# Xinjie-Q/Boosting-NeRV

Hardware: AMD Instinct MI355X
Metric: train frames/sec (higher is better)
Workload: dtype fp32; 1 GPU; NeRV-boost 1.5M (1489577 params, fc_dim 30) train step on a synthetic Bunny-shaped clip 132x3x720x1280: decoder fwd + Fusion10_freq + bwd + fused Adan; frames resident in HBM; global_batch=1, per_gpu_batch=1, parallelism=dp1, hipgraph=True, rccl_ranks=0, collective_in_graph=False

## Files before the change

boosting_nerv_amd/csrc/loss.hip:

```cpp
#include "common.h"
#include "launch.h"
#include <vector>
#include <math.h>
#include <string.h>
#include <map>
#include <mutex>

namespace {

constexpr int NSB = 512;

__device__ __forceinline__ void diff_stats_body(const float* __restrict__ p, const float* __restrict__ t, float* __restrict__ part, int n_per_sample, const int bx, const int b) {
    const float* pp = p + (size_t)b * n_per_sample;
    const float* tt = t + (size_t)b * n_per_sample;
    float s1 = 0.f, s2 = 0.f;
    constexpr int STR = NSB * 256;
    int i = bx * 256 + threadIdx.x;
    for (; i + 3 * STR < n_per_sample; i += 4 * STR) {
        float d[4];
#pragma unroll
        for (int u = 0; u < 4; ++u) d[u] = pp[i + u * STR] - tt[i + u * STR];
#pragma unroll
        for (int u = 0; u < 4; ++u) { s1 += fabsf(d[u]); s2 = fmaf(d[u], d[u], s2); }
    }
// ... 77 lines not shown
        const int oy = (int)(r % Ho);
        const size_t pl = r / Ho;
        const int iy = 2 * oy - ph, ix = 2 * ox - pw;
        const float* xp = x + pl * H * W;
        float s = 0.f;
#pragma unroll
        for (int dy = 0; dy < 2; ++dy)
#pragma unroll
            for (int dx = 0; dx < 2; ++dx) {
                const int yy = iy + dy, xx = ix + dx;
                if (yy >= 0 && yy < H && xx >= 0 && xx < W) s += xp[(size_t)yy * W + xx];
            }
        y[i] = 0.25f * s;
    }
}

struct PyrArgs { const float* src[2]; float* dst[2][LV]; int H[LV], W[LV]; int planes; int vec2; };
__device__ __forceinline__ void pyramid_body(const PyrArgs& a, const int bx, const int by, const int bz) {
    __shared__ float s1[16][17], s2[8][9], s3[4][5];
    const int img = bz & 1, pl = bz >> 1;
    const float* x = a.src[img] + (size_t)pl * a.H[0] * a.W[0];
    const int tid = threadIdx.x, ty = tid >> 4, tx = tid & 15;
    {
        const int oy = by * 16 + ty, ox = bx * 16 + tx;
        float v = 0.f;
        if (oy < a.H[1] && ox < a.W[1]) {
            const float* p0 = x + (size_t)(2 * oy) * a.W[0] + 2 * ox;
            const float* p1 = p0 + a.W[0];
            float2 r0, r1;
            if (a.vec2) {
                r0 = *reinterpret_cast<const float2*>(p0);
                r1 = *reinterpret_cast<const float2*>(p1);
            } else {
                r0 = float2{p0[0], p0[1]};
                r1 = float2{p1[0], p1[1]};
            }
            v = 0.25f * (((r0.x + r0.y) + r1.x) + r1.y);
            a.dst[img][1][((size_t)pl * a.H[1] + oy) * a.W[1] + ox] = v;
        }
        s1[ty][tx] = v;
    }
    __syncthreads();
    if (tid < 64) {
        const int y = tid >> 3, xx = tid & 7, oy = by * 8 + y, ox = bx * 8 + xx;
        const float v = 0.25f * (((s1[2 * y][2 * xx] + s1[2 * y][2 * xx + 1]) + s1[2 * y + 1][2 * xx]) + s1[2 * y + 1][2 * xx + 1]);
        if (oy < a.H[2] && ox < a.W[2]) a.dst[img][2][((size_t)pl * a.H[2] + oy) * a.W[2] + ox] = v;
        s2[y][xx] = v;
    }
    __syncthreads();
    if (tid < 16) {
        const int y = tid >> 2, xx = tid & 3, oy = by * 4 + y, ox = bx * 4 + xx;
        const float v = 0.25f * (((s2[2 * y][2 * xx] + s2[2 * y][2 * xx + 1]) + s2[2 * y + 1][2 * xx]) + s2[2 * y + 1][2 * xx + 1]);
        if (oy < a.H[3] && ox < a.W[3]) a.dst[img][3][((size_t)pl * a.H[3] + oy) * a.W[3] + ox] = v;
        s3[y][xx] = v;
    }
    __syncthreads();
    if (tid < 4) {
        const int y = tid >> 1, xx = tid & 1, oy = by * 2 + y, ox = bx * 2 + xx;
        const float v = 0.25f * (((s3[2 * y][2 * xx] + s3[2 * y][2 * xx + 1]) + s3[2 * y + 1][2 * xx]) + s3[2 * y + 1][2 * xx + 1]);
        if (oy < a.H[4] && ox < a.W[4]) a.dst[img][4][((size_t)pl * a.H[4] + oy) * a.W[4] + ox] = v;
    }
}
__global__ __launch_bounds__(256) void pyramid_kernel(const PyrArgs a) { pyramid_body(a, blockIdx.x, blockIdx.y, blockIdx.z); }

struct SsimArgs {
    const float* X; const float* Y;
    float* partial;
    const float* coef;
    float coef_k;
    const float* dcoarse;
    float* dX;
    float* G;
    int H, W, Hc, Wc, ph, pw;
    int tiles_x, tiles_y;
    float C1, C2;
    float k_l1, k_l2;
    int acc;
    Win win;
};

typedef float pk2 __attribute__((ext_vector_type(2)));
__device__ __forceinline__ pk2 pk_fma(pk2 a, pk2 b, pk2 c) { return __builtin_elementwise_fma(a, b, c); }

__device__ __forceinline__ void ssim_fwd_body(const SsimArgs& a, const bool LAST, const int bx, const int by, const int bc, const int nbc) {
#pragma clang fp contract(off)
    constexpr int WH = STH + HW_, WW = STW + HW_;
    __shared__ pk2 sXY[WH][WW];
    __shared__ pk2 sV01[STH][WW], sV23[STH][WW];
    __shared__ float sV4[STH][WW];
    __shared__ float red[4];
    const int tid = threadIdx.x;
    const int oy0 = by * STH, ox0 = bx * STW;
    const float* X = a.X + (size_t)bc * a.H * a.W;
    const float* Y = a.Y + (size_t)bc * a.H * a.W;
    {
        constexpr int NLD = (WH * WW + 255) / 256;
        pk2 ld[NLD];
#pragma unroll
        for (int u = 0; u < NLD; ++u) {
            const int i = tid + u * 256;
            const int r = i / WW, c = i - r * WW;
            const int y = oy0 + r, x = ox0 + c;
            const bool in = i < WH * WW && y < a.H && x < a.W;
            ld[u] = pk2{in ? X[(size_t)y * a.W + x] : 0.f, in ? Y[(size_t)y * a.W + x] : 0.f};
        }
#pragma unroll
        for (int u = 0; u < NLD; ++u) {
            const int i = tid + u * 256;
            if (i < WH * WW) (&sXY[0][0])[i] = ld[u];
        }
    }
    __syncthreads();
    for (int i = tid; i < STH * WW; i += 256) {
        const int r = i / WW, c = i - r * WW;
        pk2 v01 = {0.f, 0.f}, v23 = {0.f, 0.f};
        float v4 = 0.f;
#pragma unroll
        for (int k = 0; k < WS_; ++k) {
            const float g = a.win.g[k];
            const pk2 gg = {g, g}, xy = sXY[r + k][c];
            v01 = pk_fma(gg, xy, v01); v23 = pk_fma(gg, xy * xy, v23); v4 = fmaf(g, xy.x * xy.y, v4);
        }
        sV01[r][c] = v01; sV23[r][c] = v23; sV4[r][c] = v4;
    }
    __syncthreads();
    float acc = 0.f;
    const int Hv = a.H - HW_, Wv = a.W - HW_;
    for (int i = tid; i < STH * STW; i += 256) {
        const int r = i / STW, c = i - r * STW;
        pk2 m = {0.f, 0.f}, e = {0.f, 0.f};
        float exy = 0.f;
#pragma unroll
        for (int k = 0; k < WS_; ++k) {
            const float g = a.win.g[k];
            const pk2 gg = {g, g};
            m = pk_fma(gg, sV01[r][c + k], m); e = pk_fma(gg, sV23[r][c + k], e); exy = fmaf(g, sV4[r][c + k], exy);
        }
        const float m1 = m.x, m2 = m.y, exx = e.x, eyy = e.y;
        if (oy0 + r < Hv && ox0 + c < Wv) {
            const float m11 = m1 * m1, m22 = m2 * m2, m12 = m1 * m2;
            const float s1 = exx - m11, s2 = eyy - m22, s12 = exy - m12;
            const float B2 = s1 + s2 + a.C2;
            const float cs = (2.f * s12 + a.C2) / B2;
            float lum = 1.f;
            if (LAST) { lum = (2.f * m12 + a.C1) / (m11 + m22 + a.C1); acc += lum * cs; }
            else acc += cs;
            if (a.G) {
                const float dxy0 = 2.f * __builtin_amdgcn_rcpf(B2);
                float dm = dxy0 * (m1 * cs - m2), dxx = -0.5f * cs * dxy0, dxy = dxy0;
                if (LAST) {
                    const float B1 = m11 + m22 + a.C1;
                    dm = (2.f * __builtin_amdgcn_rcpf(B1)) * (m2 - m1 * lum) * cs + lum * dm;
                    dxx *= lum; dxy *= lum;
                }
                const size_t plane = (size_t)a.H * a.W, o = (size_t)bc * plane + (size_t)(oy0 + r) * a.W + (ox0 + c);
                const size_t mstride = (size_t)nbc * plane;
                a.G[o] = dm; a.G[mstride + o] = dxx; a.G[2 * mstride + o] = dxy;
            }
        }
    }
    acc = wave_sum(acc);
    if ((tid & 63) == 0) red[tid >> 6] = acc;
    __syncthreads();
    if (tid == 0) a.partial[(size_t)bc * (a.tiles_x * a.tiles_y) + by * a.tiles_x + bx] = red[0] + red[1] + red[2] + red[3];
}
struct Tile3 { int x, y, z; };
__device__ __forceinline__ Tile3 xcd_tile3() {
    const int gx = (int)gridDim.x, gy = (int)gridDim.y;
    const int lb = xcd_remap((int)(blockIdx.x + gridDim.x * (blockIdx.y + gridDim.y * blockIdx.z)), (int)(gridDim.x * gridDim.y * gridDim.z));
    const int z = lb / (gx * gy), r = lb - z * (gx * gy);
    return Tile3{r % gx, r / gx, z};
}
template <bool LAST>
__global__ __launch_bounds__(256) void ssim_fwd_kernel(const SsimArgs a) { const Tile3 t = xcd_tile3(); ssim_fwd_body(a, LAST, t.x, t.y, t.z, gridDim.z); }

struct SsimAllArgs { SsimArgs lv[LV]; int first[LV + 1]; };
__global__ __launch_bounds__(256) void ssim_fwd_all_kernel(const SsimAllArgs a) {
    const int lb = xcd_remap((int)(blockIdx.x + gridDim.x * blockIdx.y), (int)(gridDim.x * gridDim.y));
    const int gbx = lb % (int)gridDim.x, gby = lb / (int)gridDim.x;
    int l = 0;
#pragma unroll
    for (int k = 1; k < LV; ++k) if (gbx >= a.first[k]) l = k;
    const int t = gbx - a.first[l];
    const int bx = t % a.lv[l].tiles_x, by = t / a.lv[l].tiles_x;
    ssim_fwd_body(a.lv[l], l == LV - 1, bx, by, gby, gridDim.y);
}

struct CoefArgs {
    const float* partial[LV];
    int tiles[LV];
    float inv_nvalid[LV];
    float weights[LV];
    float* msval;
    float* coef;
    int BC;
    float chain;
};
__device__ __forceinline__ double tile_sum_d(const float* __restrict__ part, const int nt) {
    const int lane = threadIdx.x & 63;
    double s = 0.0;
    for (int i0 = lane; i0 < nt; i0 += 8 * 64) {
        float v[8];
#pragma unroll
        for (int u = 0; u < 8; ++u) { const int i = i0 + u * 64; v[u] = i < nt ? part[i] : 0.f; }
#pragma unroll
        for (int u = 0; u < 8; ++u) if (i0 + u * 64 < nt) s += (double)v[u];
    }
    return wave_sum_d(s);
}
__device__ __forceinline__ void ms_coef_body(const CoefArgs& a, const int bc) {
    const int lane = threadIdx.x & 63, nw = (int)blockDim.x >> 6;
    __shared__ float stat[LV];
    for (int l = threadIdx.x >> 6; l < LV; l += nw) {
        const double s = tile_sum_d(a.partial[l] + (size_t)bc * a.tiles[l], a.tiles[l]);
        if (lane == 0) stat[l] = (float)(s * (double)a.inv_nvalid[l]);
    }
    __syncthreads();
    if (threadIdx.x == 0) {
        float P = 1.f;
        for (int k = 0; k < LV; ++k) P *= powf(fmaxf(stat[k], 0.f), a.weights[k]);
        a.msval[bc] = P;
        for (int k = 0; k < LV; ++k)
            a.coef[(size_t)k * a.BC + bc] = stat[k] > 0.f ? a.chain * a.weights[k] * (P / stat[k]) * a.inv_nvalid[k] : 0.f;
    }
}
__global__ __launch_bounds__(320) void ms_coef_kernel(const CoefArgs a) { ms_coef_body(a, blockIdx.x); }

struct CoarseChain { const float* own[LV]; int H[LV], W[LV], ph[LV], pw[LV]; int n; };
constexpr int SSIM_BWD_LDS = 3 * (2 * STH + HW_) * (STW + HW_);
template <bool LEVEL0>
__device__ __forceinline__ void ssim_bwd_body(const SsimArgs& a, const CoarseChain* cc, float* lds, const int bx, const int by, const int bc, const int nbc) {
    constexpr int GH = STH + HW_, GW = STW + HW_;
    pk2 (*sG01)[GW] = reinterpret_cast<pk2 (*)[GW]>(lds);
    pk2 (*sA01)[GW] = reinterpret_cast<pk2 (*)[GW]>(lds + 2 * GH * GW);
    float (*sG2)[GW] = reinterpret_cast<float (*)[GW]>(lds + 2 * GH * GW + 2 * STH * GW);
    float (*sA2)[GW] = reinterpret_cast<float (*)[GW]>(lds + 3 * GH * GW + 2 * STH * GW);
    const int tid = threadIdx.x;
    const int py0 = by * STH, px0 = bx * STW;
    const int wy0 = py0 - HW_, wx0 = px0 - HW_;
    const int Hv = a.H - HW_, Wv = a.W - HW_;
    const size_t plane = (size_t)a.H * a.W, mstride = (size_t)nbc * plane;
    const float* Gp = a.G + (size_t)bc * plane;
    {
        constexpr int NLD = (GH * GW + 255) / 256;
        float l0[NLD], l1[NLD], l2[NLD];
#pragma unroll
        for (int u = 0; u < NLD; ++u) {
            const int i = tid + u * 256;
            const int r = i / GW, c = i - r * GW;
            const int oy = wy0 + r, ox = wx0 + c;
            l0[u] = 0.f; l1[u] = 0.f; l2[u] = 0.f;
            if (i < GH * GW && oy >= 0 && oy < Hv && ox >= 0 && ox < Wv) {
                const size_t o = (size_t)oy * a.W + ox;
                l0[u] = Gp[o]; l1[u] = Gp[mstride + o]; l2[u] = Gp[2 * mstride + o];
            }
        }
#pragma unroll
        for (int u = 0; u < NLD; ++u) {
            const int i = tid + u * 256;
            if (i < GH * GW) { (&sG01[0][0])[i] = pk2{l0[u], l1[u]}; (&sG2[0][0])[i] = l2[u]; }
        }
    }
    __syncthreads();
    for (int i = tid; i < STH * GW; i += 256) {
        const int r = i / GW, c = i - r * GW;
        pk2 a01 = {0.f, 0.f};
        float a2 = 0.f;
#pragma unroll
// ... 40 lines not shown
        }
        if (LEVEL0) {
            const float df = xv - yv;
            const float sg = (df > 0.f) ? 1.f : ((df < 0.f) ? -1.f : 0.f);
            d += a.k_l1 * sg + a.k_l2 * df;
        }
        float* dst = a.dX + ((size_t)bc * a.H + y) * a.W + x;
        *dst = (LEVEL0 && a.acc) ? d + *dst : d;
    }
}
template <bool LEVEL0>
__global__ __launch_bounds__(256) void ssim_bwd_from_g_kernel(const SsimArgs a) {
    __shared__ __attribute__((aligned(16))) float sl[SSIM_BWD_LDS];
    const Tile3 t = xcd_tile3(); ssim_bwd_body<LEVEL0>(a, nullptr, sl, t.x, t.y, t.z, gridDim.z);
}
__global__ __launch_bounds__(256) void ssim_bwd_level0_chain_kernel(const SsimArgs a, const CoarseChain cc) {
    __shared__ __attribute__((aligned(16))) float sl[SSIM_BWD_LDS];
    const Tile3 t = xcd_tile3(); ssim_bwd_body<true>(a, &cc, sl, t.x, t.y, t.z, gridDim.z);
}
__device__ __forceinline__ void ssim_bwd_coarse_body(const SsimAllArgs& a, float* lds, const int lin, const int gx, const int nbc) {
    const int lb = xcd_remap(lin, gx * nbc);
    const int gbx = lb % gx, gby = lb / gx;
    int l = 1;
#pragma unroll
    for (int k = 2; k < LV; ++k) if (gbx >= a.first[k]) l = k;
    const int t = gbx - a.first[l];
    const int tx = cdiv_d(a.lv[l].W, STW);
    ssim_bwd_body<false>(a.lv[l], nullptr, lds, t % tx, t / tx, gby, nbc);
}
__global__ __launch_bounds__(256) void ssim_bwd_coarse_all_kernel(const SsimAllArgs a) {
    __shared__ __attribute__((aligned(16))) float sl[SSIM_BWD_LDS];
    ssim_bwd_coarse_body(a, sl, (int)(blockIdx.x + gridDim.x * blockIdx.y), (int)gridDim.x, (int)gridDim.y);
}

#include "fft_body.h"
__global__ __launch_bounds__(256) void fft_rows_fwd_kernel(const FftArgs a) { fft_rows_fwd_body(a, blockIdx.x); }
__global__ __launch_bounds__(256) void fft_cols_kernel(const FftArgs a) {
    const int lb = xcd_remap((int)(blockIdx.x + gridDim.x * blockIdx.y), (int)(gridDim.x * gridDim.y));
    fft_cols_body(a, lb % (int)gridDim.x, lb / (int)gridDim.x, gridDim.x);
}
__global__ __launch_bounds__(256) void fft_rows_adj_kernel(const FftArgs a) { fft_rows_adj_body(a, blockIdx.x); }

struct FinalArgs {
    const float* stats_part;
    const float* msval;
    const float* fft_part;
    float* loss_out; float* stats_out;
    int B, C, n_per_sample, ncolblk;
    float c_l1, c_l2, c_ms, c_fft;
};
__device__ __forceinline__ void loss_final_body(const FinalArgs& a) {
    const int lane = threadIdx.x;
    double total = 0.0;
    for (int b = 0; b < a.B; ++b) {
        double s1 = 0.0, s2 = 0.0;
        for (int k = lane; k < NSB; k += 64) { s1 += (double)a.stats_part[((size_t)b * NSB + k) * 2]; s2 += (double)a.stats_part[((size_t)b * NSB + k) * 2 + 1]; }
        s1 = wave_sum_d(s1); s2 = wave_sum_d(s2);
        double l = (double)a.c_l1 * (s1 / a.n_per_sample) + (double)a.c_l2 * (s2 / a.n_per_sample);
        double ms = 0.0;
        if (a.msval) {
            for (int c = 0; c < a.C; ++c) ms += (double)a.msval[b * a.C + c];
            ms /= a.C;
            l += (double)a.c_ms * (1.0 - ms);
        }
        if (a.fft_part) {
            double f = 0.0;
            const int nf = a.C * a.ncolblk;
            for (int k = lane; k < nf; k += 64) f += (double)a.fft_part[(size_t)b * nf + k];
            f = wave_sum_d(f);
            l += (double)a.c_fft * f / (2.0 * (double)a.n_per_sample);
        }
        if (lane == 0) {
            float* so = a.stats_out + b * BNERV_LOSS_STATS;
            so[0] = (float)l; so[1] = (float)s1; so[2] = (float)s2; so[3] = (float)ms;
            const float mse = (float)(s2 / (double)a.n_per_sample);
            so[4] = -10.0f * log10f(mse + 1e-9f);
        }
        total += l;
    }
    if (lane == 0) a.loss_out[0] = (float)(total / a.B);
}
__global__ __launch_bounds__(64) void loss_final_kernel(const FinalArgs a) { loss_final_body(a); }

struct LossHeadArgs { FftArgs f; PyrArgs p; const float* pred; const float* target; float* stats_part; int nps, n_fft, n_pyr, pyr_gx, pyr_gy; };
__global__ __launch_bounds__(256) void loss_head_kernel(const LossHeadArgs a) {
    int b = blockIdx.x;
    if (b < a.n_fft) { fft_rows_fwd_body(a.f, b); return; }
    b -= a.n_fft;
    if (b < a.n_pyr) { const int bx = b % a.pyr_gx, r = b / a.pyr_gx; pyramid_body(a.p, bx, r % a.pyr_gy, r / a.pyr_gy); return; }
    b -= a.n_pyr;
    diff_stats_body(a.pred, a.target, a.stats_part, a.nps, b % NSB, b / NSB);
}
struct LossMidArgs { FftArgs f; CoefArgs c; int ncolblk, n_cols; };
__global__ __launch_bounds__(256) void loss_mid_kernel(const LossMidArgs a) {
    const int b = blockIdx.x;
    if (b < a.n_cols) {
        const int xcd = b & 7, k = b >> 3, per = a.n_cols >> 3, extra = a.n_cols & 7;
        const int lb = xcd * per + min(xcd, extra) + k;
        fft_cols_body(a.f, lb % a.ncolblk, lb / a.ncolblk, a.ncolblk);
    } else ms_coef_body(a.c, b - a.n_cols);
}
struct LossTailArgs { SsimArgs s; CoarseChain cc; FinalArgs fin; int gx, gy, n0, BC; };
__global__ __launch_bounds__(256) void loss_tail_kernel(const LossTailArgs a) {
    __shared__ __attribute__((aligned(16))) float sl[SSIM_BWD_LDS];
    if ((int)blockIdx.x < a.n0) { const int b = xcd_remap((int)blockIdx.x, a.n0); const int bx = b % a.gx, r = b / a.gx; ssim_bwd_body<true>(a.s, &a.cc, sl, bx, r % a.gy, r / a.gy, a.BC); }
    else if (threadIdx.x < 64) loss_final_body(a.fin);
}
struct LossCoarseArgs { FftArgs f; SsimAllArgs s; int n_adj, gx, BC; };
__global__ __launch_bounds__(256) void loss_coarse_kernel(const LossCoarseArgs a) {
    extern __shared__ __attribute__((aligned(16))) float sm[];
    const int b = blockIdx.x;
    if (b < a.n_adj) { fft_rows_adj_body(a.f, b); return; }
    ssim_bwd_coarse_body(a.s, sm, b - a.n_adj, a.gx, a.BC);
}
__global__ void msssim_final_kernel(const float* __restrict__ msval, float* __restrict__ out, int B, int C) {
    const int b = blockIdx.x * blockDim.x + threadIdx.x;
    if (b >= B) return;
    float s = 0.f;
    for (int c = 0; c < C; ++c) s += msval[b * C + c];
    out[b] = s / C;
}


__device__ __forceinline__ void ssim_plane_body(const float* __restrict__ part, const int nt, const float inv_nvalid, float* val, const int bc) {
    const double s = tile_sum_d(part + (size_t)bc * nt, nt);
    if ((threadIdx.x & 63) == 0) val[bc] = (float)(s * (double)inv_nvalid);
}
struct SsimFinalArgs { const float* part; float* val; float inv_nvalid; int tiles, BC; FinalArgs fin; };
__device__ __forceinline__ void ssim_planes_body(const SsimFinalArgs& a) {
    const int nw = (int)blockDim.x >> 6;
    for (int bc = threadIdx.x >> 6; bc < a.BC; bc += nw) ssim_plane_body(a.part, a.tiles, a.inv_nvalid, a.val, bc);
    __threadfence();
    __syncthreads();
}
__device__ __forceinline__ void ssim_final_body(const SsimFinalArgs& a) {
    ssim_planes_body(a);
    if (threadIdx.x < 64) loss_final_body(a.fin);
}
__global__ __launch_bounds__(256) void ssim_final_kernel(const SsimFinalArgs a) { ssim_final_body(a); }

constexpr int SSIM_FFT_MAX_RADIX = 37;
__global__ __launch_bounds__(256) void ssim_fft_cols_kernel(const FftArgs a) {
    const int lb = xcd_remap((int)(blockIdx.x + gridDim.x * blockIdx.y), (int)(gridDim.x * gridDim.y));
    fft_cols_body<SSIM_FFT_MAX_RADIX>(a, lb % (int)gridDim.x, lb / (int)gridDim.x, gridDim.x);
}
__global__ __launch_bounds__(256) void ssim_fft_rows_fwd_kernel(const FftArgs a) { fft_rows_fwd_body<SSIM_FFT_MAX_RADIX>(a, blockIdx.x); }
__global__ __launch_bounds__(256) void ssim_fft_rows_adj_kernel(const FftArgs a) { fft_rows_adj_body<SSIM_FFT_MAX_RADIX>(a, blockIdx.x); }

struct SsimHeadArgs { SsimArgs s; const float* pred; const float* target; float* stats_part; int nps, n_sums, BC; };
__global__ __launch_bounds__(256) void ssim_head_kernel(const SsimHeadArgs a) {
    int b = blockIdx.x;
    if (b < a.n_sums) { diff_stats_body(a.pred, a.target, a.stats_part, a.nps, b % NSB, b / NSB); return; }
    b -= a.n_sums;
    const int nt = a.s.tiles_x * a.s.tiles_y;
    const int t = xcd_remap(b, nt * a.BC);
    const int bc = t / nt, r = t - bc * nt;
    ssim_fwd_body(a.s, true, r % a.s.tiles_x, r / a.s.tiles_x, bc, a.BC);
}

struct SsimTailArgs { SsimArgs s; SsimFinalArgs fin; int gx, gy, n0, BC; };
__global__ __launch_bounds__(256) void ssim_tail_kernel(const SsimTailArgs a) {
    __shared__ __attribute__((aligned(16))) float sl[SSIM_BWD_LDS];
    if ((int)blockIdx.x < a.n0) { const int b = xcd_remap((int)blockIdx.x, a.n0); const int bx = b % a.gx, r = b / a.gx; ssim_bwd_body<true>(a.s, nullptr, sl, bx, r % a.gy, r / a.gy, a.BC); }
    else ssim_final_body(a.fin);
}
__global__ __launch_bounds__(256) void ssim_metric_kernel(const SsimFinalArgs a, float* __restrict__ out, int B, int C) {
    ssim_planes_body(a);
    for (int b = threadIdx.x; b < B; b += blockDim.x) {
        double ms = 0.0;
        for (int c = 0; c < C; ++c) ms += (double)a.val[b * C + c];
        ms /= C;
        out[b] = (float)ms;
    }
}

constexpr float SSIM_C1 = 0.01f * 0.01f, SSIM_C2 = 0.03f * 0.03f;
constexpr float MS_WEIGHTS[LV] = {0.0448f, 0.2856f, 0.3001f, 0.2363f, 0.1333f};

struct WsLayout {
    size_t stats_part, pyrX[LV], pyrY[LV], dXl[LV], Gl[LV], ssim_part[LV], msval, coef, T, fft_part, total;
    int tiles_x[LV], tiles_y[LV], tiles[LV];
    Pyr pyr;
    int ncolblk, BC;
};
static size_t align64(size_t x) { return (x + 63) & ~size_t(63); }
static WsLayout make_layout(int B, int C, int H, int W, int levels, bool use_fft) {
    WsLayout L{};
    size_t off = 0;
    auto take = [&](size_t n) { size_t o = off; off = align64(off + n); return o; };
    const size_t BC = (size_t)B * C;
    L.BC = (int)BC;
    L.stats_part = take((size_t)B * NSB * 2);
    if (levels) L.pyr = make_pyr(H, W);
    for (int l = 0; l < levels; ++l) {
        const size_t n = BC * L.pyr.H[l] * L.pyr.W[l];
        if (l > 0) { L.pyrX[l] = take(n); L.pyrY[l] = take(n); L.dXl[l] = take(n); }
        L.Gl[l] = take(3 * n);
        L.tiles_x[l] = cdiv(L.pyr.W[l] - HW_, STW); L.tiles_y[l] = cdiv(L.pyr.H[l] - HW_, STH); L.tiles[l] = L.tiles_y[l] * L.tiles_x[l];
        L.ssim_part[l] = take(BC * L.tiles[l]);
    }
    if (levels) L.msval = take(BC);
    if (levels == LV) L.coef = take(BC * LV);
    if (use_fft) {
        L.ncolblk = cdiv(W / 2 + 1, COLS_PER_BLOCK);
        L.T = take(BC * H * (size_t)(W / 2 + 1) * 2);
        L.fft_part = take(BC * L.ncolblk);
    }
    L.total = off;
    return L;
}

static SsimArgs level_args(const float* X, const float* Y, float* grad, float* ws, const WsLayout& L, int l) {
    static const Win win = make_win();
    SsimArgs a{};
    a.X = l ? ws + L.pyrX[l] : X; a.Y = l ? ws + L.pyrY[l] : Y; a.dX = l ? ws + L.dXl[l] : grad; a.G = ws + L.Gl[l];
    a.partial = ws + L.ssim_part[l]; a.coef = ws + L.coef + (size_t)l * L.BC;
    a.H = L.pyr.H[l]; a.W = L.pyr.W[l]; a.tiles_x = L.tiles_x[l]; a.tiles_y = L.tiles_y[l];
    a.C1 = SSIM_C1; a.C2 = SSIM_C2; a.win = win;
    return a;
}
static float inv_nvalid(const WsLayout& L, int l) { return 1.0f / ((float)(L.pyr.H[l] - HW_) * (float)(L.pyr.W[l] - HW_)); }

static CoefArgs coef_args(float* ws, const WsLayout& L, float chain) {
    CoefArgs ca{};
    for (int l = 0; l < LV; ++l) { ca.partial[l] = ws + L.ssim_part[l]; ca.tiles[l] = L.tiles[l]; ca.inv_nvalid[l] = inv_nvalid(L, l); ca.weights[l] = MS_WEIGHTS[l]; }
    ca.msval = ws + L.msval; ca.coef = ws + L.coef; ca.BC = L.BC; ca.chain = chain;
    return ca;
}
static int ms_forward_args(const float* X, const float* Y, float* ws, const WsLayout& L, bool want_g, PyrArgs& pa, SsimAllArgs& sa) {
    pa.src[0] = X; pa.src[1] = Y; pa.planes = L.BC;
    pa.vec2 = ((reinterpret_cast<uintptr_t>(X) | reinterpret_cast<uintptr_t>(Y)) & 7) == 0 ? 1 : 0;
    int nblk = 0;
    for (int l = 0; l < LV; ++l) {
        pa.H[l] = L.pyr.H[l]; pa.W[l] = L.pyr.W[l];
        if (L.pyr.H[l] <= HW_ || L.pyr.W[l] <= HW_) return bnerv_set_error(BNERV_E_ARG, "ms_ssim: level %d is %dx%d, needs > %d on both sides", l, L.pyr.H[l], L.pyr.W[l], HW_);
        if (l > 0) { pa.dst[0][l] = ws + L.pyrX[l]; pa.dst[1][l] = ws + L.pyrY[l]; }
        sa.lv[l] = level_args(X, Y, nullptr, ws, L, l);
        if (!want_g) sa.lv[l].G = nullptr;
        sa.first[l] = nblk;
        nblk += L.tiles[l];
// ... 80 lines not shown
static int run_ms_forward(hipStream_t st, const float* X, const float* Y, float* ws, const WsLayout& L, float chain, bool want_g) {
    PyrArgs pa{}; SsimAllArgs sa{};
    int rc = ms_forward_args(X, Y, ws, L, want_g, pa, sa);
    if (rc) return rc;
    if (even_pyramid(L)) {
        hipLaunchKernelGGL(pyramid_kernel, dim3(cdiv(L.pyr.W[1], 16), cdiv(L.pyr.H[1], 16), 2 * L.BC), dim3(256), 0, st, pa);
        BNERV_LAUNCH_CHECK("pyramid");
    } else { rc = launch_pools(st, X, Y, ws, L); if (rc) return rc; }
    if (loss_fused()) {
        hipLaunchKernelGGL(ssim_fwd_all_kernel, dim3(sa.first[LV], L.BC), dim3(256), 0, st, sa);
        BNERV_LAUNCH_CHECK("ssim_fwd_all");
    } else {
        for (int l = 0; l < LV; ++l) {
            const dim3 grid(sa.lv[l].tiles_x, sa.lv[l].tiles_y, L.BC);
            if (l == LV - 1) hipLaunchKernelGGL(ssim_fwd_kernel<true>, grid, dim3(256), 0, st, sa.lv[l]);
            else hipLaunchKernelGGL(ssim_fwd_kernel<false>, grid, dim3(256), 0, st, sa.lv[l]);
            BNERV_LAUNCH_CHECK("ssim_fwd");
        }
    }
    hipLaunchKernelGGL(ms_coef_kernel, dim3(L.BC), dim3(320), 0, st, coef_args(ws, L, chain));
    BNERV_LAUNCH_CHECK("ms_coef");
    return BNERV_OK;
}

static int run_ms_backward(hipStream_t st, const float* X, const float* Y, float* grad, float* ws, const WsLayout& L, float k_l1, float k_l2, int acc) {
    if (loss_fused()) {
        SsimAllArgs sa{};
        CoarseChain cc{};
        ms_backward_args(X, Y, grad, ws, L, k_l1, k_l2, acc, sa, cc);
        hipLaunchKernelGGL(ssim_bwd_coarse_all_kernel, dim3(sa.first[LV], L.BC), dim3(256), 0, st, sa);
        BNERV_LAUNCH_CHECK("ssim_bwd_coarse_all");
        hipLaunchKernelGGL(ssim_bwd_level0_chain_kernel, dim3(cdiv(L.pyr.W[0], STW), cdiv(L.pyr.H[0], STH), L.BC), dim3(256), 0, st, sa.lv[0], cc);
        BNERV_LAUNCH_CHECK("ssim_bwd_level0");
        return BNERV_OK;
    }
    for (int l = LV - 1; l >= 0; --l) {
        SsimArgs a = level_args(X, Y, grad, ws, L, l);
        if (l < LV - 1) { a.dcoarse = ws + L.dXl[l + 1]; a.Hc = L.pyr.H[l + 1]; a.Wc = L.pyr.W[l + 1]; a.ph = a.H % 2; a.pw = a.W % 2; }
        if (l == 0) { a.k_l1 = k_l1; a.k_l2 = k_l2; a.acc = acc; }
        const dim3 grid(cdiv(a.W, STW), cdiv(a.H, STH), L.BC);
        if (l == 0) hipLaunchKernelGGL((ssim_bwd_from_g_kernel<true>), grid, dim3(256), 0, st, a);
        else hipLaunchKernelGGL((ssim_bwd_from_g_kernel<false>), grid, dim3(256), 0, st, a);
        BNERV_LAUNCH_CHECK("ssim_bwd");
    }
    return BNERV_OK;
}

static int launch_stats(hipStream_t st, const float* p, const float* t, float* part, int B, int n_per_sample) {
    hipLaunchKernelGGL(diff_stats_kernel, dim3(NSB, B), dim3(256), 0, st, p, t, part, n_per_sample);
    BNERV_LAUNCH_CHECK("diff_stats");
    return BNERV_OK;
}

}

extern "C" size_t bnerv_loss_ws_bytes(int B, int C, int H, int W, int use_ms, int use_fft) {
    if (B <= 0 || C <= 0 || H <= 0 || W <= 0) return 0;
    return make_layout(B, C, H, W, use_ms ? LV : 0, use_fft != 0).total * sizeof(float);
}

extern "C" int bnerv_loss_fwd_bwd(void* stream, const bnerv_loss_desc* dp) {
    LossCall c;
    if (const int rc_d = open_loss_call(dp, "loss", c)) return rc_d;
    const bnerv_loss_desc& d = c.d;
    const bool use_ms = d.c_ms != 0.f, use_fft = d.c_fft != 0.f;
    const WsLayout L = make_layout(d.B, d.C, d.H, d.W, use_ms ? LV : 0, use_fft);
    if (d.ws_bytes < L.total * sizeof(float)) return bnerv_set_error(BNERV_E_WS, "loss: workspace %zu < %zu", d.ws_bytes, L.total * sizeof(float));
    hipStream_t st = (hipStream_t)stream;
    float* ws = reinterpret_cast<float*>(d.ws);
    const int BC = c.BC;
    if (use_ms && (d.H <= 160 || d.W <= 160)) return bnerv_set_error(BNERV_E_ARG, "loss: MS-SSIM needs min(H,W) > 160 (got %dx%d)", d.H, d.W);
    FftLaunch F{};
    if (use_fft) {
        if (const int rc_f = fft_launch_args(c, ws, L, BNERV_FFT_MAX_RADIX, 160 * 1024, false, "loss", F)) return rc_f;
        F.a.accumulate = 1;
    }
    const FinalArgs f = final_args(c, ws, L, use_ms ? ws + L.msval : nullptr, d.c_ms);
    const float chain = -d.c_ms / (float)BC;

    const bool late = adj_late();
    if (use_ms && use_fft && d.grad && loss_fused() && loss_merged()) {
        const bool even = even_pyramid(L);
        LossHeadArgs ha{}; LossMidArgs ma{}; LossTailArgs ta{};
        SsimAllArgs sf{};
        int rc = ms_forward_args(d.pred, d.target, ws, L, true, ha.p, sf);
        if (rc) return rc;
        ha.f = F.a; ha.pred = d.pred; ha.target = d.target; ha.stats_part = ws + L.stats_part; ha.nps = c.nps;
        ha.n_fft = F.nrowblk; ha.pyr_gx = cdiv(L.pyr.W[1], 16); ha.pyr_gy = cdiv(L.pyr.H[1], 16); ha.n_pyr = even ? ha.pyr_gx * ha.pyr_gy * 2 * BC : 0;
        if (const int rc_lds = dyn_lds<&loss_head_kernel>(F.lds_row, "loss_head")) return rc_lds;
        hipLaunchKernelGGL(loss_head_kernel, dim3(ha.n_fft + ha.n_pyr + NSB * d.B), dim3(256), F.lds_row, st, ha);
        BNERV_LAUNCH_CHECK("loss_head");
        if (!even) { rc = launch_pools(st, d.pred, d.target, ws, L); if (rc) return rc; }
        hipLaunchKernelGGL(ssim_fwd_all_kernel, dim3(sf.first[LV], BC), dim3(256), 0, st, sf);
        BNERV_LAUNCH_CHECK("ssim_fwd_all");
        ma.f = F.a; ma.c = coef_args(ws, L, chain); ma.ncolblk = L.ncolblk; ma.n_cols = L.ncolblk * BC;
        if (const int rc_lds = dyn_lds<&loss_mid_kernel>(F.lds_col, "loss_mid")) return rc_lds;
        hipLaunchKernelGGL(loss_mid_kernel, dim3(ma.n_cols + BC), dim3(256), F.lds_col, st, ma);
        BNERV_LAUNCH_CHECK("loss_mid");
        SsimAllArgs sb{};
        ms_backward_args(d.pred, d.target, d.grad, ws, L, c.k_l1, c.k_l2, late ? 0 : 1, sb, ta.cc);
        if (late) {
            hipLaunchKernelGGL(ssim_bwd_coarse_all_kernel, dim3(sb.first[LV], BC), dim3(256), 0, st, sb);
            BNERV_LAUNCH_CHECK("ssim_bwd_coarse_all");
        } else {
            LossCoarseArgs ca{};
            ca.f = F.a; ca.f.accumulate = 0; ca.s = sb; ca.n_adj = F.nrowblk; ca.gx = sb.first[LV]; ca.BC = BC;
            const size_t lds_c = F.lds_row > SSIM_BWD_LDS * sizeof(float) ? F.lds_row : SSIM_BWD_LDS * sizeof(float);
            if (const int rc_lds = dyn_lds<&loss_coarse_kernel>(lds_c, "loss_coarse")) return rc_lds;
            hipLaunchKernelGGL(loss_coarse_kernel, dim3(ca.n_adj + ca.gx * BC), dim3(256), lds_c, st, ca);
            BNERV_LAUNCH_CHECK("loss_coarse");
        }
        ta.s = sb.lv[0]; ta.fin = f; ta.gx = cdiv(L.pyr.W[0], STW); ta.gy = cdiv(L.pyr.H[0], STH); ta.BC = BC; ta.n0 = ta.gx * ta.gy * BC;
        hipLaunchKernelGGL(loss_tail_kernel, dim3(ta.n0 + 1), dim3(256), 0, st, ta);
        BNERV_LAUNCH_CHECK("loss_tail");
        if (late) {
            if (const int rc_lds = dyn_lds<&fft_rows_adj_kernel>(F.lds_row, "fft_rows_adj")) return rc_lds;
            hipLaunchKernelGGL(fft_rows_adj_kernel, dim3(F.nrowblk), dim3(256), F.lds_row, st, F.a);
            BNERV_LAUNCH_CHECK("fft_rows_adj");
        }
        return BNERV_OK;
    }

    const bool fft_first = use_ms && use_fft && d.grad && !late;
    int rc = launch_stats(st, d.pred, d.target, ws + L.stats_part, d.B, c.nps);
    if (rc) return rc;
    auto run_fft = [&](int accumulate) -> int {
        FftArgs fa = F.a; fa.accumulate = accumulate;
        if (const int rc_lds = dyn_lds<&fft_rows_fwd_kernel>(F.lds_row, "fft_rows_fwd")) return rc_lds;
        if (const int rc_lds = dyn_lds<&fft_rows_adj_kernel>(F.lds_row, "fft_rows_adj")) return rc_lds;
        if (const int rc_lds = dyn_lds<&fft_cols_kernel>(F.lds_col, "fft_cols")) return rc_lds;
        hipLaunchKernelGGL(fft_rows_fwd_kernel, dim3(F.nrowblk), dim3(256), F.lds_row, st, fa);
        BNERV_LAUNCH_CHECK("fft_rows_fwd");
        hipLaunchKernelGGL(fft_cols_kernel, dim3(L.ncolblk, BC), dim3(256), F.lds_col, st, fa);
        BNERV_LAUNCH_CHECK("fft_cols");
        if (d.grad) {
            hipLaunchKernelGGL(fft_rows_adj_kernel, dim3(F.nrowblk), dim3(256), F.lds_row, st, fa);
            BNERV_LAUNCH_CHECK("fft_rows_adj");
        }
        return BNERV_OK;
    };
    if (use_ms) {
        rc = run_ms_forward(st, d.pred, d.target, ws, L, chain, d.grad != nullptr);
        if (rc) return rc;
        if (fft_first) { rc = run_fft(0); if (rc) return rc; }
        if (d.grad) { rc = run_ms_backward(st, d.pred, d.target, d.grad, ws, L, c.k_l1, c.k_l2, fft_first ? 1 : 0); if (rc) return rc; }
    } else if (d.grad) {
        const size_t n = (size_t)d.B * c.nps;
        int gx = (int)((n + 1023) / 1024); if (gx > 4096) gx = 4096;
        hipLaunchKernelGGL(grad_l1l2_kernel, dim3(gx), dim3(256), 0, st, d.pred, d.target, d.grad, n, c.k_l1, c.k_l2);
        BNERV_LAUNCH_CHECK("grad_l1l2");
    }
    if (use_fft && !fft_first) { rc = run_fft(1); if (rc) return rc; }
    hipLaunchKernelGGL(loss_final_kernel, dim3(1), dim3(64), 0, st, f);
    BNERV_LAUNCH_CHECK("loss_final");
    return BNERV_OK;
}

extern "C" int bnerv_msssim(void* stream, const float* x, const float* y, float* out, void* wsv, size_t ws_bytes, int B, int C, int H, int W) {
    BNERV_REQUIRE(x && y && out && wsv && B > 0 && C > 0, "msssim: bad args");
    if (H <= 160 || W <= 160) return bnerv_set_error(BNERV_E_ARG, "msssim: needs min(H,W) > 160 (got %dx%d)", H, W);
    const WsLayout L = make_layout(B, C, H, W, LV, false);
    if (ws_bytes < L.total * sizeof(float)) return bnerv_set_error(BNERV_E_WS, "msssim: workspace %zu < %zu", ws_bytes, L.total * sizeof(float));
    hipStream_t st = (hipStream_t)stream;
    float* ws = reinterpret_cast<float*>(wsv);
    int rc = run_ms_forward(st, x, y, ws, L, 0.f, false);
    if (rc) return rc;
    hipLaunchKernelGGL(msssim_final_kernel, dim3(cdiv(B, 64)), dim3(64), 0, st, ws + L.msval, out, B, C);
    BNERV_LAUNCH_CHECK("msssim_final");
    return BNERV_OK;
}

extern "C" size_t bnerv_loss_ssim_ws_bytes(int B, int C, int H, int W, int use_fft) {
    if (B <= 0 || C <= 0 || H <= HW_ || W <= HW_) return 0;
    return make_layout(B, C, H, W, 1, use_fft != 0).total * sizeof(float);
}

extern "C" int bnerv_loss_ssim_fwd_bwd(void* stream, const bnerv_loss_desc* dp, float c_ssim) {
    LossCall c;
    if (const int rc_d = open_loss_call(dp, "loss_ssim", c)) return rc_d;
    const bnerv_loss_desc& d = c.d;
    BNERV_REQUIRE(d.c_ms == 0.f, "loss_ssim: c_ms must be 0 (the MS-SSIM losses go through bnerv_loss_fwd_bwd)");
    BNERV_REQUIRE(c_ssim != 0.f, "loss_ssim: c_ssim is 0 (losses without an SSIM term go through bnerv_loss_fwd_bwd)");
    if (d.H <= HW_ || d.W <= HW_) return bnerv_set_error(BNERV_E_ARG, "loss_ssim: SSIM needs min(H,W) >= %d (got %dx%d)", WS_, d.H, d.W);
    const bool use_fft = d.c_fft != 0.f;
    const WsLayout L = make_layout(d.B, d.C, d.H, d.W, 1, use_fft);
    if (d.ws_bytes < L.total * sizeof(float)) return bnerv_set_error(BNERV_E_WS, "loss_ssim: workspace %zu < %zu", d.ws_bytes, L.total * sizeof(float));
    hipStream_t st = (hipStream_t)stream;
    float* ws = reinterpret_cast<float*>(d.ws);
    const int BC = c.BC;
    BNERV_REQUIRE((size_t)L.tiles[0] * BC + (size_t)BC * d.H + (size_t)NSB * d.B < (size_t)1 << 30, "loss_ssim: batch too large for one grid");
    FftLaunch F{};
    if (use_fft) {
        if (const int rc_f = fft_launch_args(c, ws, L, SSIM_FFT_MAX_RADIX, 128 * 1024, true, "loss_ssim", F)) return rc_f;
        if (const int rc_lds = dyn_lds<&ssim_fft_rows_fwd_kernel>(F.lds_row, "ssim_fft_rows_fwd")) return rc_lds;
// ... 80 lines not shown
```

Measured before the change: 691.2 frames/s.

## Repartition merged loss kernels: fold level-0 SSIM fwd into head, coarse levels into mid

The full-resolution SSIM forward tiles now run in the loss head kernel beside the row FFT, pyramid and diff-stats blocks. The coarser pyramid levels run in the mid kernel next to the column FFT, which removes the separate ssim_fwd_all launch and lets that work overlap the FFT. ms_coef moves into a new kernel that shares its launch with the adjoint row FFT. The coarse SSIM backward becomes its own launch. SSIM forward LDS is moved to a caller-provided buffer so the bodies can share dynamic shared memory, which raises LDS per block for the head and mid kernels and may lower their occupancy.

```diff
diff --git a/boosting_nerv_amd/csrc/loss.hip b/boosting_nerv_amd/csrc/loss.hip
--- a/boosting_nerv_amd/csrc/loss.hip
+++ b/boosting_nerv_amd/csrc/loss.hip
@@ -183,13 +183,15 @@
 typedef float pk2 __attribute__((ext_vector_type(2)));
 __device__ __forceinline__ pk2 pk_fma(pk2 a, pk2 b, pk2 c) { return __builtin_elementwise_fma(a, b, c); }
 
-__device__ __forceinline__ void ssim_fwd_body(const SsimArgs& a, const bool LAST, const int bx, const int by, const int bc, const int nbc) {
+constexpr int SSIM_FWD_LDS = 2 * (STH + HW_) * (STW + HW_) + 5 * STH * (STW + HW_) + 4;
+__device__ __forceinline__ void ssim_fwd_body(const SsimArgs& a, float* lds, const bool LAST, const int bx, const int by, const int bc, const int nbc) {
 #pragma clang fp contract(off)
     constexpr int WH = STH + HW_, WW = STW + HW_;
-    __shared__ pk2 sXY[WH][WW];
-    __shared__ pk2 sV01[STH][WW], sV23[STH][WW];
-    __shared__ float sV4[STH][WW];
-    __shared__ float red[4];
+    pk2 (*sXY)[WW] = reinterpret_cast<pk2 (*)[WW]>(lds);
+    pk2 (*sV01)[WW] = reinterpret_cast<pk2 (*)[WW]>(lds + 2 * WH * WW);
+    pk2 (*sV23)[WW] = reinterpret_cast<pk2 (*)[WW]>(lds + 2 * WH * WW + 2 * STH * WW);
+    float (*sV4)[WW] = reinterpret_cast<float (*)[WW]>(lds + 2 * WH * WW + 4 * STH * WW);
+    float* red = lds + 2 * WH * WW + 5 * STH * WW;
     const int tid = threadIdx.x;
     const int oy0 = by * STH, ox0 = bx * STW;
     const float* X = a.X + (size_t)bc * a.H * a.W;
@@ -273,18 +275,25 @@
     return Tile3{r % gx, r / gx, z};
 }
 template <bool LAST>
-__global__ __launch_bounds__(256) void ssim_fwd_kernel(const SsimArgs a) { const Tile3 t = xcd_tile3(); ssim_fwd_body(a, LAST, t.x, t.y, t.z, gridDim.z); }
+__global__ __launch_bounds__(256) void ssim_fwd_kernel(const SsimArgs a) {
+    __shared__ __attribute__((aligned(16))) float sl[SSIM_FWD_LDS];
+    const Tile3 t = xcd_tile3(); ssim_fwd_body(a, sl, LAST, t.x, t.y, t.z, gridDim.z);
+}
 
 struct SsimAllArgs { SsimArgs lv[LV]; int first[LV + 1]; };
-__global__ __launch_bounds__(256) void ssim_fwd_all_kernel(const SsimAllArgs a) {
-    const int lb = xcd_remap((int)(blockIdx.x + gridDim.x * blockIdx.y), (int)(gridDim.x * gridDim.y));
-    const int gbx = lb % (int)gridDim.x, gby = lb / (int)gridDim.x;
-    int l = 0;
+__device__ __forceinline__ void ssim_fwd_levels_body(const SsimAllArgs& a, float* lds, const int l0, const int lin, const int gx, const int nbc) {
+    const int lb = xcd_remap(lin, gx * nbc);
+    const int gbx = a.first[l0] + lb % gx, gby = lb / gx;
+    int l = l0;
 #pragma unroll
     for (int k = 1; k < LV; ++k) if (gbx >= a.first[k]) l = k;
     const int t = gbx - a.first[l];
     const int bx = t % a.lv[l].tiles_x, by = t / a.lv[l].tiles_x;
-    ssim_fwd_body(a.lv[l], l == LV - 1, bx, by, gby, gridDim.y);
+    ssim_fwd_body(a.lv[l], lds, l == LV - 1, bx, by, gby, nbc);
+}
+__global__ __launch_bounds__(256) void ssim_fwd_all_kernel(const SsimAllArgs a) {
+    __shared__ __attribute__((aligned(16))) float sl[SSIM_FWD_LDS];
+    ssim_fwd_levels_body(a, sl, 0, (int)(blockIdx.x + gridDim.x * blockIdx.y), (int)gridDim.x, (int)gridDim.y);
 }
 
 struct CoefArgs {
@@ -491,36 +500,45 @@
 }
 __global__ __launch_bounds__(64) void loss_final_kernel(const FinalArgs a) { loss_final_body(a); }
 
-struct LossHeadArgs { FftArgs f; PyrArgs p; const float* pred; const float* target; float* stats_part; int nps, n_fft, n_pyr, pyr_gx, pyr_gy; };
+struct LossHeadArgs { FftArgs f; SsimArgs s; PyrArgs p; const float* pred; const float* target; float* stats_part; int nps, n_fft, n_s0, BC, n_pyr, pyr_gx, pyr_gy; };
 __global__ __launch_bounds__(256) void loss_head_kernel(const LossHeadArgs a) {
+    extern __shared__ __attribute__((aligned(16))) float sm[];
     int b = blockIdx.x;
     if (b < a.n_fft) { fft_rows_fwd_body(a.f, b); return; }
     b -= a.n_fft;
+    if (b < a.n_s0) {
+        const int nt = a.s.tiles_x * a.s.tiles_y;
+        const int t = xcd_remap(b, a.n_s0);
+        const int bc = t / nt, r = t - bc * nt;
+        ssim_fwd_body(a.s, sm, false, r % a.s.tiles_x, r / a.s.tiles_x, bc, a.BC);
+        return;
+    }
+    b -= a.n_s0;
     if (b < a.n_pyr) { const int bx = b % a.pyr_gx, r = b / a.pyr_gx; pyramid_body(a.p, bx, r % a.pyr_gy, r / a.pyr_gy); return; }
     b -= a.n_pyr;
     diff_stats_body(a.pred, a.target, a.stats_part, a.nps, b % NSB, b / NSB);
 }
-struct LossMidArgs { FftArgs f; CoefArgs c; int ncolblk, n_cols; };
+struct LossMidArgs { FftArgs f; SsimAllArgs s; int ncolblk, n_cols, gx, BC; };
 __global__ __launch_bounds__(256) void loss_mid_kernel(const LossMidArgs a) {
+    extern __shared__ __attribute__((aligned(16))) float sm[];
     const int b = blockIdx.x;
     if (b < a.n_cols) {
         const int xcd = b & 7, k = b >> 3, per = a.n_cols >> 3, extra = a.n_cols & 7;
         const int lb = xcd * per + min(xcd, extra) + k;
         fft_cols_body(a.f, lb % a.ncolblk, lb / a.ncolblk, a.ncolblk);
-    } else ms_coef_body(a.c, b - a.n_cols);
+    } else ssim_fwd_levels_body(a.s, sm, 1, b - a.n_cols, a.gx, a.BC);
+}
+struct LossCoefArgs { FftArgs f; CoefArgs c; int n_adj; };
+__global__ __launch_bounds__(256) void loss_coef_kernel(const LossCoefArgs a) {
+    const int b = blockIdx.x;
+    if (b < a.n_adj) fft_rows_adj_body(a.f, b);
+    else ms_coef_body(a.c, b - a.n_adj);
 }
 struct LossTailArgs { SsimArgs s; CoarseChain cc; FinalArgs fin; int gx, gy, n0, BC; };
 __global__ __launch_bounds__(256) void loss_tail_kernel(const LossTailArgs a) {
     __shared__ __attribute__((aligned(16))) float sl[SSIM_BWD_LDS];
     if ((int)blockIdx.x < a.n0) { const int b = xcd_remap((int)blockIdx.x, a.n0); const int bx = b % a.gx, r = b / a.gx; ssim_bwd_body<true>(a.s, &a.cc, sl, bx, r % a.gy, r / a.gy, a.BC); }
     else if (threadIdx.x < 64) loss_final_body(a.fin);
-}
-struct LossCoarseArgs { FftArgs f; SsimAllArgs s; int n_adj, gx, BC; };
-__global__ __launch_bounds__(256) void loss_coarse_kernel(const LossCoarseArgs a) {
-    extern __shared__ __attribute__((aligned(16))) float sm[];
-    const int b = blockIdx.x;
-    if (b < a.n_adj) { fft_rows_adj_body(a.f, b); return; }
-    ssim_bwd_coarse_body(a.s, sm, b - a.n_adj, a.gx, a.BC);
 }
 __global__ void msssim_final_kernel(const float* __restrict__ msval, float* __restrict__ out, int B, int C) {
     const int b = blockIdx.x * blockDim.x + threadIdx.x;
@@ -558,13 +576,14 @@
 
 struct SsimHeadArgs { SsimArgs s; const float* pred; const float* target; float* stats_part; int nps, n_sums, BC; };
 __global__ __launch_bounds__(256) void ssim_head_kernel(const SsimHeadArgs a) {
+    __shared__ __attribute__((aligned(16))) float sl[SSIM_FWD_LDS];
     int b = blockIdx.x;
     if (b < a.n_sums) { diff_stats_body(a.pred, a.target, a.stats_part, a.nps, b % NSB, b / NSB); return; }
     b -= a.n_sums;
     const int nt = a.s.tiles_x * a.s.tiles_y;
     const int t = xcd_remap(b, nt * a.BC);
     const int bc = t / nt, r = t - bc * nt;
-    ssim_fwd_body(a.s, true, r % a.s.tiles_x, r / a.s.tiles_x, bc, a.BC);
+    ssim_fwd_body(a.s, sl, true, r % a.s.tiles_x, r / a.s.tiles_x, bc, a.BC);
 }
 
 struct SsimTailArgs { SsimArgs s; SsimFinalArgs fin; int gx, gy, n0, BC; };
@@ -811,34 +830,37 @@
     if (use_ms && use_fft && d.grad && loss_fused() && loss_merged()) {
         const bool even = even_pyramid(L);
         LossHeadArgs ha{}; LossMidArgs ma{}; LossTailArgs ta{};
-        SsimAllArgs sf{};
-        int rc = ms_forward_args(d.pred, d.target, ws, L, true, ha.p, sf);
+        int rc = ms_forward_args(d.pred, d.target, ws, L, true, ha.p, ma.s);
         if (rc) return rc;
-        ha.f = F.a; ha.pred = d.pred; ha.target = d.target; ha.stats_part = ws + L.stats_part; ha.nps = c.nps;
-        ha.n_fft = F.nrowblk; ha.pyr_gx = cdiv(L.pyr.W[1], 16); ha.pyr_gy = cdiv(L.pyr.H[1], 16); ha.n_pyr = even ? ha.pyr_gx * ha.pyr_gy * 2 * BC : 0;
-        if (const int rc_lds = dyn_lds<&loss_head_kernel>(F.lds_row, "loss_head")) return rc_lds;
-        hipLaunchKernelGGL(loss_head_kernel, dim3(ha.n_fft + ha.n_pyr + NSB * d.B), dim3(256), F.lds_row, st, ha);
+        BNERV_REQUIRE((size_t)ma.s.first[LV] * BC + (size_t)BC * d.H + (size_t)NSB * d.B < (size_t)1 << 30, "loss: batch too large for one grid");
+        const size_t lds_s = SSIM_FWD_LDS * sizeof(float);
+        ha.f = F.a; ha.s = ma.s.lv[0]; ha.pred = d.pred; ha.target = d.target; ha.stats_part = ws + L.stats_part; ha.nps = c.nps;
+        ha.n_fft = F.nrowblk; ha.n_s0 = L.tiles[0] * BC; ha.BC = BC;
+        ha.pyr_gx = cdiv(L.pyr.W[1], 16); ha.pyr_gy = cdiv(L.pyr.H[1], 16); ha.n_pyr = even ? ha.pyr_gx * ha.pyr_gy * 2 * BC : 0;
+        const size_t lds_h = F.lds_row > lds_s ? F.lds_row : lds_s;
+        if (const int rc_lds = dyn_lds<&loss_head_kernel>(lds_h, "loss_head")) return rc_lds;
+        hipLaunchKernelGGL(loss_head_kernel, dim3(ha.n_fft + ha.n_s0 + ha.n_pyr + NSB * d.B), dim3(256), lds_h, st, ha);
         BNERV_LAUNCH_CHECK("loss_head");
         if (!even) { rc = launch_pools(st, d.pred, d.target, ws, L); if (rc) return rc; }
-        hipLaunchKernelGGL(ssim_fwd_all_kernel, dim3(sf.first[LV], BC), dim3(256), 0, st, sf);
-        BNERV_LAUNCH_CHECK("ssim_fwd_all");
-        ma.f = F.a; ma.c = coef_args(ws, L, chain); ma.ncolblk = L.ncolblk; ma.n_cols = L.ncolblk * BC;
-        if (const int rc_lds = dyn_lds<&loss_mid_kernel>(F.lds_col, "loss_mid")) return rc_lds;
-        hipLaunchKernelGGL(loss_mid_kernel, dim3(ma.n_cols + BC), dim3(256), F.lds_col, st, ma);
+        ma.f = F.a; ma.ncolblk = L.ncolblk; ma.n_cols = L.ncolblk * BC; ma.gx = ma.s.first[LV] - ma.s.first[1]; ma.BC = BC;
+        const size_t lds_m = F.lds_col > lds_s ? F.lds_col : lds_s;
+        if (const int rc_lds = dyn_lds<&loss_mid_kernel>(lds_m, "loss_mid")) return rc_lds;
+        hipLaunchKernelGGL(loss_mid_kernel, dim3(ma.n_cols + ma.gx * BC), dim3(256), lds_m, st, ma);
         BNERV_LAUNCH_CHECK("loss_mid");
+        if (late) {
+            hipLaunchKernelGGL(ms_coef_kernel, dim3(BC), dim3(320), 0, st, coef_args(ws, L, chain));
+            BNERV_LAUNCH_CHECK("ms_coef");
+        } else {
+            LossCoefArgs ca{};
+            ca.f = F.a; ca.f.accumulate = 0; ca.c = coef_args(ws, L, chain); ca.n_adj = F.nrowblk;
+            if (const int rc_lds = dyn_lds<&loss_coef_kernel>(F.lds_row, "loss_coef")) return rc_lds;
+            hipLaunchKernelGGL(loss_coef_kernel, dim3(ca.n_adj + BC), dim3(256), F.lds_row, st, ca);
+            BNERV_LAUNCH_CHECK("loss_coef");
+        }
         SsimAllArgs sb{};
         ms_backward_args(d.pred, d.target, d.grad, ws, L, c.k_l1, c.k_l2, late ? 0 : 1, sb, ta.cc);
-        if (late) {
-            hipLaunchKernelGGL(ssim_bwd_coarse_all_kernel, dim3(sb.first[LV], BC), dim3(256), 0, st, sb);
-            BNERV_LAUNCH_CHECK("ssim_bwd_coarse_all");
-        } else {
-            LossCoarseArgs ca{};
-            ca.f = F.a; ca.f.accumulate = 0; ca.s = sb; ca.n_adj = F.nrowblk; ca.gx = sb.first[LV]; ca.BC = BC;
-            const size_t lds_c = F.lds_row > SSIM_BWD_LDS * sizeof(float) ? F.lds_row : SSIM_BWD_LDS * sizeof(float);
-            if (const int rc_lds = dyn_lds<&loss_coarse_kernel>(lds_c, "loss_coarse")) return rc_lds;
-            hipLaunchKernelGGL(loss_coarse_kernel, dim3(ca.n_adj + ca.gx * BC), dim3(256), lds_c, st, ca);
-            BNERV_LAUNCH_CHECK("loss_coarse");
-        }
+        hipLaunchKernelGGL(ssim_bwd_coarse_all_kernel, dim3(sb.first[LV], BC), dim3(256), 0, st, sb);
+        BNERV_LAUNCH_CHECK("ssim_bwd_coarse_all");
         ta.s = sb.lv[0]; ta.fin = f; ta.gx = cdiv(L.pyr.W[0], STW); ta.gy = cdiv(L.pyr.H[0], STH); ta.BC = BC; ta.n0 = ta.gx * ta.gy * BC;
         hipLaunchKernelGGL(loss_tail_kernel, dim3(ta.n0 + 1), dim3(256), 0, st, ta);
         BNERV_LAUNCH_CHECK("loss_tail");
```

Result: no change. 693.0 frames/s, median of 2 (+0.3%).
